# dfm/george

Measured on NVIDIA H100. Metric: gp.compute+log_likelihood N-points/sec, higher is better.
Workload: dtype f64

## Files before the change

george_b200/csrc/hodlr.cu:

```cuda
#include <algorithm>
#include <cmath>
#include <cstdlib>
#include <cstring>
#include <vector>

#include "common.cuh"
#include "hodlr_kernels.cuh"
#include "hodlr_lu.cuh"
#include "hodlr_aca2.cuh"
#include "hodlr_leaf.cuh"
#include "linalg.cuh"
#include "kernel_eval.cuh"

namespace bgp {
int upload_program(const DevProgram& P, DevBuf<DevProgram>& buf, cudaStream_t s);
int kmat_grad_contract_launch(const DevProgram* dprog, int nd, int np, const unsigned* which_dev, const double* x,
                              int64_t n, const double* M, int64_t ldm, const double* alpha, double ca, double cm,
                              double* g_dev, double* diag_dev, DevBuf<double>& scratch, cudaStream_t s);
int fill_identity_launch(double* A, int64_t n, cudaStream_t s);
int64_t grad_slab_partial_size(int64_t n, int64_t c, int np);
int64_t grad_slab_tile_size(int64_t n, int np);
int kmat_grad_slab_launch(const DevProgram* dprog, int nd, int np, const unsigned* which_dev, const double* x, int64_t n,
                          const double* W, int64_t j0, int64_t nc, int64_t jlo, int64_t jhi, const double* alpha,
                          double* partial, double* tile_part, double* diag_dev, cudaStream_t s);
// ... 94 lines not shown
  DevBuf<int> d_idx, d_piv_rows, d_piv_cols, d_ticket, d_chain_done, d_ncols_by_depth;
  DevBuf<uint32_t> d_chain_state;
  DevBuf<A2Node> d_a2nodes;
  DevBuf<A2State> d_a2states;
  DevBuf<MT19937> d_a2rngs;
  DevBuf<A2EPart> d_epart;
  DevBuf<int> d_cand, d_cand_k, d_cand_words, d_cand_L, d_cand_next, d_cand_live, d_cchunk_node, d_rchunk_node, d_nactive;
  DevBuf<double> d_node_box;
  DevBuf<double2> d_cand_xu, d_gbox, d_cbox;
  DevBuf<unsigned long long> d_cmax, d_stats;
  DevBuf<int4> d_work;
  DevBuf<int> d_work_count, d_iter;
  AcaGraphKey aca_key;
  cudaGraph_t aca_graph = nullptr;
  cudaGraphExec_t aca_exec = nullptr;
  cudaStream_t sC = nullptr;
  bool profile = false;
  std::vector<cudaEvent_t> prof_events;
  double prof[12] = {0, 0, 0, 0, 0, 0, 0, 0, 0, 0, 0, 0};
  uint64_t draw_paths[4] = {0, 0, 0, 0};
  uint64_t eval_units[2] = {0, 0};
  DevBuf<double> d_vpart, d_upart, d_vmax;
  int aca_iters = 0;
  size_t w_cap = 0;

  double t_ms[5] = {0, 0, 0, 0, 0};
  double grad_t[4] = {0, 0, 0, 0};
  double work[6] = {0, 0, 0, 0, 0, 0};
};

static int ensure_streams(bgp_hodlr* h) {
  if (!h->sA) {
    BGP_CUDA(cudaStreamCreateWithFlags(&h->sA, cudaStreamNonBlocking));
    BGP_CUDA(cudaStreamCreateWithFlags(&h->sB, cudaStreamNonBlocking));
    for (int i = 0; i < 8; ++i) BGP_CUDA(cudaEventCreate(&h->ev[i]));
  }
  return BGP_OK;
}

static void build_tree(bgp_hodlr* h, int start, int size, int dir, int parent, int depth) {
  HNode nd;
  nd.start = start; nd.size = size; nd.half = size / 2; nd.dir = dir; nd.parent = parent; nd.depth = depth;
  nd.is_leaf = !(nd.half >= h->opts.min_size);
  nd.slot = 0;
  const int id = (int)h->nodes.size();
  h->nodes.push_back(nd);
  if (!nd.is_leaf) {
    build_tree(h, start, nd.half, 0, id, depth + 1);
    build_tree(h, start + nd.half, size - nd.half, 1, id, depth + 1);
  }
}

static int hodlr_solve_dev(bgp_hodlr* h, double* b, int64_t nrhs, int64_t ldb, cudaStream_t s, int part,
                           int64_t eye_row0 = -1);
static int hodlr_exchange_finish(bgp_hodlr* h);

static bool host_exchange(const bgp_hodlr* h) {
  return h->opts.shard_count > 1 &&
         !(comm_ready() && comm_world() == h->opts.shard_count && comm_rank() == h->opts.shard_rank);
}

static int reject_host_exchange(const bgp_hodlr* h, const char* what) {
  if (!host_exchange(h)) return BGP_OK;
  set_error("%s is not available on a host-exchange shard (shard %d of %d without a matching communicator): use "
            "bgp_hodlr_solve_local_dev / bgp_hodlr_solve_top_dev", what, h->opts.shard_rank, h->opts.shard_count);
  return BGP_ERR_INVALID;
}
// ... 198 lines not shown
  BGP_TRY(h->d_cand_L.reserve((size_t)cand_total, s));
  BGP_TRY(h->d_cand_next.reserve((size_t)cand_total, s));
  BGP_TRY(h->d_cand_live.reserve((size_t)cand_total, s));
  BGP_TRY(h->d_node_box.reserve((size_t)2 * nn, s));
  BGP_TRY(h->d_cmax.reserve((size_t)cand_total, s));
  BGP_TRY(h->d_epart.reserve((size_t)std::max(ncc, 1) * A2_NSUB, s));
  BGP_TRY(h->d_cchunk_node.reserve(ncc, s));
  BGP_TRY(h->d_rchunk_node.reserve(nrc, s));
  BGP_TRY(h->d_vpart.reserve((size_t)ncc * A2_NSUB * (capmax + 1), s));
  BGP_TRY(h->d_upart.reserve((size_t)nrc * A2_NSUB * (capmax + 1), s));
  const bool cull = shape_has_bound(h->prog.shape) && !getenv("BGP_NO_CULL");
  if (cull) {
    BGP_TRY(h->d_vmax.reserve((size_t)ncc * A2_NGROUP, s));
    BGP_TRY(h->d_cand_xu.reserve((size_t)cand_total, s));
    BGP_TRY(h->d_gbox.reserve((size_t)ncc * A2_NGROUP, s));
    BGP_TRY(h->d_cbox.reserve((size_t)ncc, s));
  }
  BGP_TRY(h->d_nactive.reserve(2, s));
  int n_top = 0;
  for (int i = 0; i < nn; ++i) n_top += hn[i].is_top;
  BGP_TRY(h->d_stats.reserve(A2_NSTATS, s));
  int64_t work_cap = 0;
  for (int i = 0; i < nn; ++i) {
    const int big = (hn[i].bmax + A2_CG * A2_ITEM_CB - 1) / (A2_CG * A2_ITEM_CB);
    const int small = (std::min(hn[i].bmax, 256) + A2_CG - 1) / A2_CG;
    work_cap += (int64_t)hn[i].n_cchunks * std::max(big, small);
  }
  BGP_TRY(h->d_work.reserve((size_t)(2 * work_cap), s));
  BGP_TRY(h->d_work_count.reserve(4, s));
  BGP_TRY(h->d_iter.reserve(1, s));
  BGP_CUDA(cudaMemsetAsync(h->d_iter.p, 0, sizeof(int), s));
  BGP_CUDA(cudaMemsetAsync(h->d_work_count.p, 0, sizeof(int) * 4, s));
  BGP_CUDA(cudaMemsetAsync(h->d_stats.p, 0, sizeof(unsigned long long) * A2_NSTATS, s));
  BGP_CUDA(cudaMemcpyAsync(h->d_a2nodes.p, hn.data(), sizeof(A2Node) * nn, cudaMemcpyHostToDevice, s));
  BGP_CUDA(cudaMemcpyAsync(h->d_cchunk_node.p, cchunk_node.data(), sizeof(int) * ncc, cudaMemcpyHostToDevice, s));
  BGP_CUDA(cudaMemcpyAsync(h->d_rchunk_node.p, rchunk_node.data(), sizeof(int) * nrc, cudaMemcpyHostToDevice, s));
  BGP_CUDA(cudaMemcpyAsync(h->d_nactive.p, &nn, sizeof(int), cudaMemcpyHostToDevice, s));
  A2Args a;
  memset(&a, 0, sizeof(a));
  a.prog = h->d_prog.p; a.x = h->d_x.p; a.nodes = h->d_a2nodes.p; a.states = h->d_a2states.p; a.rngs = h->d_a2rngs.p; a.n_nodes = nn;
  a.tol = h->opts.tol; a.seed = (uint32_t)h->opts.seed; a.exhaust_mode = h->opts.exhaust_mode;
  a.idx_ws = h->d_idx.p; a.piv_rows = h->d_piv_rows.p; a.piv_cols = h->d_piv_cols.p;
  a.cand = h->d_cand.p; a.cand_k = h->d_cand_k.p; a.cand_words = h->d_cand_words.p; a.cmax = h->d_cmax.p; a.epart = h->d_epart.p;
  a.cchunk_node = h->d_cchunk_node.p; a.rchunk_node = h->d_rchunk_node.p; a.vpart = h->d_vpart.p; a.upart = h->d_upart.p;
  a.vmax = cull ? h->d_vmax.p : nullptr;
  a.cand_xu = cull ? h->d_cand_xu.p : nullptr;
  a.gbox = cull ? h->d_gbox.p : nullptr;
  a.cbox = cull ? h->d_cbox.p : nullptr;
  a.cand_L = h->d_cand_L.p; a.cand_next = h->d_cand_next.p; a.cand_live = h->d_cand_live.p; a.node_box = h->d_node_box.p;
  a.capmax = capmax; a.n_active = h->d_nactive.p; a.stats = h->d_stats.p;
  a.work = h->d_work.p; a.work_count = h->d_work_count.p; a.work_cursor = h->d_work_count.p + 2; a.work_cap = (int)work_cap; a.iter_ptr = h->d_iter.p;
  a.shard_rank = dist_top ? h->opts.shard_rank : 0; a.shard_count = dist_top ? h->opts.shard_count : 1;
  if (dist_top) BGP_CUDA(cudaMemcpyAsync(h->d_nactive.p + 1, &n_top, sizeof(int), cudaMemcpyHostToDevice, s));
  cudaFuncSetAttribute(a2_init_kernel, cudaFuncAttributeMaxDynamicSharedMemorySize, (int)sizeof(A2NodeSmem));
    cudaFuncSetAttribute(a2_decide_kernel, cudaFuncAttributeMaxDynamicSharedMemorySize, (int)sizeof(A2NodeSmem));
    cudaFuncSetAttribute(a2_finish_kernel, cudaFuncAttributeMaxDynamicSharedMemorySize, (int)sizeof(A2NodeSmem));
  a2_init_kernel<<<nn, A2_NODE_THREADS, sizeof(A2NodeSmem), s>>>(a);
  BGP_LAUNCH_CHECK();
  int active = nn, iters = 0;
  int eval_minb = A2_EVAL_MINB_DEFAULT;
  if (const char* e = getenv("BGP_EVAL_MINB")) eval_minb = atoi(e) == 3 ? 3 : 2;
  const int eval_grid = num_sms() * 6;
  auto launch_iteration = [&](cudaStream_t st, cudaGraphConditionalHandle hnd, int use_hnd, int it_prof) -> int {
    auto mark = [&](int slot) -> int {
      if (it_prof < 0) return BGP_OK;
      const size_t need = (size_t)7 * (it_prof + 1);
      while (h->prof_events.size() < need) {
        cudaEvent_t e;
        BGP_CUDA(cudaEventCreate(&e));
        h->prof_events.push_back(e);
      }
      BGP_CUDA(cudaEventRecord(h->prof_events[(size_t)7 * it_prof + slot], st));
      return BGP_OK;
    };
    BGP_TRY(mark(0));
    a2_eval_launch(h->prog.shape, dim3(eval_grid), st, a, eval_minb);
    BGP_LAUNCH_CHECK();
    BGP_TRY(mark(1));
    a2_decide_kernel<<<nn, A2_NODE_THREADS, sizeof(A2NodeSmem), st>>>(a);
    BGP_LAUNCH_CHECK();
    BGP_TRY(mark(2));
    a2_vrow_launch(h->prog.shape, dim3(ncc, A2_NSUB), st, a);
    BGP_LAUNCH_CHECK();
    BGP_TRY(mark(3));
    a2_pivot_kernel<<<nn, 32, 0, st>>>(a);
    BGP_LAUNCH_CHECK();
    BGP_TRY(mark(4));
    a2_vnorm_ucol_launch(h->prog.shape, dim3(ncc + nrc, A2_NSUB), st, a, ncc);
    BGP_LAUNCH_CHECK();
// ... 195 lines not shown
    hleaves[i].start = nd.start; hleaves[i].size = nd.size; hleaves[i].depth = nd.depth; hleaves[i]._pad = 0;
    hleaves[i].off = loff;
    loff += (int64_t)nd.size * nd.size;
    h->max_leaf = std::max(h->max_leaf, nd.size);
  }
  if (h->max_leaf > LS_MAX_LEAF) {
    set_error("leaf size %d too large: the leaf solve handles at most %d rows (N=%lld, min_size=%d); lower min_size",
              h->max_leaf, LS_MAX_LEAF, (long long)n, o.min_size);
    return BGP_ERR_INVALID;
  }
  BGP_TRY(h->d_leaves.reserve(std::max(nl, 1), sA));
  BGP_TRY(h->d_L.reserve((size_t)std::max<int64_t>(loff, 1), sA));
  BGP_TRY(h->d_leaf_logdet.reserve(std::max(nl, 1), sA));
  if (nl) {
    BGP_CUDA(cudaMemcpyAsync(h->d_leaves.p, hleaves.data(), sizeof(LeafDesc) * nl, cudaMemcpyHostToDevice, sA));
    const char* lf_env = getenv("BGP_LEAF_FACTOR");
    const bool generic = lf_env && strcmp(lf_env, "generic") == 0;
    if (h->max_leaf <= LF_MAX_LEAF && !generic) {
      leaf_factor_launch(h->prog.shape, nl, h->max_leaf, sA, h->d_prog.p, h->d_x.p, h->d_diag.p, h->d_leaves.p, h->d_L.p,
                         h->d_leaf_logdet.p);
    } else {
      leaf_build_factor_kernel<<<nl, LEAF_THREADS, 0, sA>>>(h->d_prog.p, h->d_x.p, h->d_diag.p, h->d_leaves.p, h->d_L.p,
                                                            h->d_leaf_logdet.p);
    }
    BGP_LAUNCH_CHECK();
  }
  BGP_CUDA(cudaEventRecord(h->ev[1], sA));

  std::vector<AcaDesc> hdesc;
  std::vector<int> desc_node;
  std::vector<AcaOut> houts;
  int64_t idx_total = 0, piv_total = 0;
  int nint = 0;
  BGP_CUDA(cudaStreamWaitEvent(sB, h->ev[1], 0));
  for (int attempt = 0;; ++attempt) {
    int vcols_set[2] = {0, 0};
    for (auto& L : h->levels) { L.vcol = vcols_set[L.set]; vcols_set[L.set] += L.cap; }
    h->top.vcols = vcols_set[0]; h->loc.vcols = vcols_set[1];
    h->vcols = vcols_set[0] + vcols_set[1];
    hdesc.clear(); desc_node.clear();
    h->piv_off.assign(h->nodes.size(), -1);
    idx_total = 0; piv_total = 0; nint = 0;
    for (int l = 0; l < nlev; ++l) {
      for (int id : h->levels[l].nodes) {
        const HNode& nd = h->nodes[id];
        AcaDesc d;
        d.row0 = nd.start + nd.half; d.n_rows = nd.size - nd.half; d.col0 = nd.start; d.n_cols = nd.half;
        d.vcol = h->levels[l].vcol; d.cap = h->levels[l].cap; d.pre_id = id; d.node = nint;
        d.idx_off = idx_total; d.piv_off = piv_total;
        h->piv_off[id] = (int)piv_total;
        idx_total += d.n_rows; piv_total += d.cap;
        hdesc.push_back(d); desc_node.push_back(id);
        nint++;
      }
    }
    std::vector<int> order(nint);
    for (int i = 0; i < nint; ++i) order[i] = i;
    if (o.rng_mode == BGP_RNG_REFERENCE) std::sort(order.begin(), order.end(), [&](int a, int b) { return hdesc[a].pre_id < hdesc[b].pre_id; });
    else std::stable_sort(order.begin(), order.end(), [&](int a, int b) {
      const int ta = h->nodes[hdesc[a].pre_id].top, tb = h->nodes[hdesc[b].pre_id].top;
      if (ta != tb) return ta > tb;
      return hdesc[a].n_rows > hdesc[b].n_rows;
    });
    std::vector<AcaDesc> hdesc_sorted(nint);
    for (int i = 0; i < nint; ++i) hdesc_sorted[i] = hdesc[order[i]];

    {
// ... 1084 lines not shown
```

george_b200/csrc/hodlr_aca2.cuh:

```cuda
#pragma once

#include "hodlr_kernels.cuh"

namespace bgp {

constexpr int A2_CHUNK = 1024;
constexpr int A2_THREADS = 256;
constexpr int A2_NODE_THREADS = 1024;
constexpr int A2_EPT = A2_CHUNK / A2_THREADS;
constexpr int A2_CG = 4;
constexpr int A2_ITEM_CB = 8;
constexpr int A2_BMAX = 8192;
constexpr int A2_EVAL_MINB_DEFAULT = 3;
constexpr int A2_BGROW = 8;
constexpr int A2_NSUB = 4;
constexpr int A2_GROUP = A2_CHUNK / (A2_THREADS / 32);
constexpr int A2_NGROUP = A2_CHUNK / A2_GROUP;
static_assert(A2_NSUB * A2_THREADS == A2_CHUNK, "sub-chunks tile a chunk");
constexpr int A2_HASH = 16384;
static_assert(A2_BMAX <= 65536, "multimap values are 16-bit draw numbers");
constexpr int A2_XWORDS = 64;
constexpr int A2_PUB_BLOCKS = A2_BMAX / (A2_CG * A2_ITEM_CB);
static_assert(256 / A2_CG <= A2_PUB_BLOCKS, "blocks of A2_CG candidates (batches of up to 256 live ones) fit too");

struct A2Node {
  int row0, n_rows, col0, n_cols;
  int vcol, cap, pre_id, node;
  int cchunk0, n_cchunks, rchunk0, n_rchunks;
  int bmax, is_top;
  int64_t idx_off, piv_off, cand_off;
  double* vbase;
  int64_t ld;
};

struct A2State {
  int rank, draws, n_index, fallback, status, active;
  int phase;
  int B, ncand, piv_i, piv_j;
  int end_words;
  int deferred;
  double pivot, norm;
// ... 90 lines not shown
  double* node_box;
  unsigned long long* cmax;
  A2EPart* epart;
  const int* cchunk_node;
  const int* rchunk_node;
  double* vpart;
  double* upart;
  double* vmax;
  double2* cand_xu;
  double2* gbox;
  double2* cbox;
  int capmax;
  int* n_active;
  int4* work;
  int* work_count;
  int* work_cursor;
  int work_cap;
  int* iter_ptr;
  int shard_rank, shard_count;
  unsigned long long* stats;
};
enum {
  A2_PATH_REDO = 4,
  A2_PATH_TRUNCATED = 5,
  A2_PATH_SEQUENTIAL = 6,
  A2_PATH_PARTIAL = 7,
  A2_UNITS_PULLED = 8,
  A2_UNITS_LIVE = 9,
  A2_NSTATS = 10
};

struct A2NodeSmem {
  MT19937 rng;
  int k[A2_BMAX];
  int ol[A2_BMAX];
  int hkey[A2_HASH];
  unsigned short hval[A2_HASH];
  uint32_t raw[A2_BMAX + A2_XWORDS];
  double red[32];
  int redi[32];
  int flag;
  int n_live;
  int extra;
};
static_assert(sizeof(int) * A2_HASH >= sizeof(double) * (3 * A2_PUB_BLOCKS + 1), "a2_generate's per-block ranges fit in hkey");

__device__ __forceinline__ unsigned a2_hash(int pos) { return ((unsigned)pos * 2654435761u) & (A2_HASH - 1); }
__device__ __forceinline__ int a2_prev_writer(const A2NodeSmem& S, int pos, int c) {
  int best = -1;
  unsigned h = a2_hash(pos);
  while (true) {
    const int key = S.hkey[h];
    if (key == -1) break;
    if (key == pos) { const int v = S.hval[h]; if (v < c && v > best) best = v; }
    h = (h + 1) & (A2_HASH - 1);
  }
  return best;
}
__device__ __forceinline__ int a2_next_writer(const A2NodeSmem& S, int pos, int c) {
  int best = 0x7fffffff;
  unsigned h = a2_hash(pos);
  while (true) {
    const int key = S.hkey[h];
    if (key == -1) break;
    if (key == pos) { const int v = S.hval[h]; if (v > c && v < best) best = v; }
    h = (h + 1) & (A2_HASH - 1);
  }
  return best;
// ... 26 lines not shown
  total = 0;
  for (int w = 0; w < nw; ++w) {
    const int t = s_warp[w];
    before += (w < warp) ? t : 0;
    total += t;
  }
  return before + inc - v;
}

__device__ inline void a2_generate(const A2Args& a, A2State& st, A2NodeSmem& S, const A2Node& nd, int nid, int nb) {
  int* __restrict__ index = a.idx_ws + nd.idx_off;
  int* __restrict__ cand = a.cand + nd.cand_off;
  int* __restrict__ cand_k = a.cand_k + nd.cand_off;
  int* __restrict__ words = a.cand_words + nd.cand_off;
  int* __restrict__ cand_L = a.cand_L + nd.cand_off;
  int* __restrict__ cand_next = a.cand_next + nd.cand_off;
  int* __restrict__ live = a.cand_live + nd.cand_off;
  unsigned long long* __restrict__ cmax = a.cmax + nd.cand_off;
  const int n_index = st.n_index;
  int B = min(min(st.B, nd.bmax), n_index);
  MT19937* rng_commit = a.rngs + 2 * (int64_t)nid;
  MT19937* rng_end = rng_commit + 1;
  if (threadIdx.x == 0) { S.flag = 0x7fffffff; S.n_live = 0; S.extra = 0; }
  mt_fill_coop(S.rng, S.raw, B);
  int start = 0;
  bool truncated = false;
  while (true) {
    const int extra = S.extra;
    for (int c = start + threadIdx.x; c < B; c += blockDim.x) {
      const uint32_t srange = (uint32_t)(n_index - c);
      const uint64_t prod = (uint64_t)S.raw[c + extra] * (uint64_t)srange;
      const uint32_t low = (uint32_t)prod;
      if (low < srange && low < (0u - srange) % srange) atomicMin(&S.flag, c);
      S.k[c] = (int)(prod >> 32);
      words[c] = c + 1 + extra;
      cmax[c] = 0ull;
    }
    __syncthreads();
    const int c0 = S.flag;
    if (c0 == 0x7fffffff) break;
    __syncthreads();
    if (threadIdx.x == 0) {
      atomicAdd(a.stats + A2_PATH_REDO, 1ull);
      const uint32_t srange = (uint32_t)(n_index - c0);
      const uint32_t thr = (0u - srange) % srange;
      int e = extra;
      int kk = -1;
      while (e + 1 < A2_XWORDS && c0 + e + 1 < B + extra) {
        ++e;
        const uint64_t prod = (uint64_t)S.raw[c0 + e] * (uint64_t)srange;
        if ((uint32_t)prod >= thr) { kk = (int)(prod >> 32); break; }
      }
      if (kk >= 0) { S.k[c0] = kk; words[c0] = c0 + 1 + e; S.extra = e; S.flag = 0x7fffffff; }
      else S.flag = -1 - c0;
    }
    __syncthreads();
    if (S.flag < 0) {
      const int c0t = -1 - S.flag;
      __syncthreads();
      if (c0t > 0) {
        if (threadIdx.x == 0) atomicAdd(a.stats + A2_PATH_TRUNCATED, 1ull);
        B = c0t; truncated = true; break;
      }
      mt_copy(&S.rng, rng_commit);
      __syncthreads();
      if (threadIdx.x == 0) {
        atomicAdd(a.stats + A2_PATH_SEQUENTIAL, 1ull);
        int w = 0; S.k[0] = mt_uniform(S.rng, (uint32_t)n_index, &w); words[0] = w; cmax[0] = 0ull; S.extra = -1;
      }
      __syncthreads();
      B = 1;
      break;
    }
    {
      const int grown = S.extra - extra;
      mt_fill_coop(S.rng, S.raw + B + extra, grown);
    }
    start = c0 + 1;
  }
  __syncthreads();
  mt_copy(rng_end, &S.rng);
  if (threadIdx.x == 0) {
    st.ncand = B;
    st.end_words = (!truncated && S.extra >= 0 && B > 0 && words[B - 1] == B + S.extra) ? B + S.extra : -1;
  }
  for (int t = threadIdx.x; t < A2_HASH; t += blockDim.x) S.hkey[t] = -1;
  __syncthreads();
  for (int c = threadIdx.x; c < B; c += blockDim.x) {
    const int pos = S.k[c];
    S.ol[c] = index[n_index - 1 - c];
    unsigned h = a2_hash(pos);
    while (atomicCAS(&S.hkey[h], -1, pos) != -1) h = (h + 1) & (A2_HASH - 1);
    S.hval[h] = (unsigned short)c;
  }
  __syncthreads();
  int* wl = reinterpret_cast<int*>(S.raw);
  for (int c = threadIdx.x; c < B; c += blockDim.x) wl[c] = a2_prev_writer(S, n_index - 1 - c, c);
  __syncthreads();
  auto last_value = [&](int c) {
    int w = wl[c];
    while (w >= 0) { c = w; w = wl[c]; }
    return S.ol[c];
  };
  for (int c = threadIdx.x; c < B; c += blockDim.x) {
    const int pos = S.k[c];
    const int wk = a2_prev_writer(S, pos, c);
    const int row = (wk < 0) ? index[pos] : last_value(wk);
    cand[c] = row;
    cand_k[c] = pos;
    cand_L[c] = last_value(c);
    cand_next[c] = a2_next_writer(S, pos, c);
  }
  const bool cull = a.vmax != nullptr;
  const int rank = st.rank;
  if (!cull) {
    for (int c = threadIdx.x; c < B; c += blockDim.x) live[c] = c;
    if (threadIdx.x == 0) S.n_live = B;
  } else {
    const double clo = a.node_box[2 * nid], chi = a.node_box[2 * nid + 1];
    const double* Ucol = nd.vbase + nd.row0;
    const double* xr = a.x + nd.row0;
    constexpr int G = 4;
    for (int t0 = 0; t0 < B; t0 += G * blockDim.x) {
      const int c0 = t0 + threadIdx.x;
      int row[G];
      double xi[G], b[G];
#pragma unroll
      for (int j = 0; j < G; ++j) { const int c = c0 + j * blockDim.x; row[j] = (c < B) ? cand[c] : 0; }
#pragma unroll
      for (int j = 0; j < G; ++j) xi[j] = xr[row[j]];
#pragma unroll
      for (int j = 0; j < G; ++j) b[j] = 0.0;
      for (int q = 0; q < rank; ++q) {
        double u[G];
#pragma unroll
        for (int j = 0; j < G; ++j) u[j] = __ldcg(Ucol + (int64_t)q * nd.ld + row[j]);
#pragma unroll
        for (int j = 0; j < G; ++j) b[j] += fabs(u[j]);
      }
      unsigned keep = 0u;
#pragma unroll
      for (int j = 0; j < G; ++j) {
        const int c = c0 + j * blockDim.x;
        if (c < B) {
          const double bb = b[j] + program_bound(a.prog, fmax(0.0, fmax(clo - xi[j], xi[j] - chi)), fmax(xi[j] - clo, chi - xi[j]));
          if (!(bb * 1.000001 < 1e-14)) keep |= 1u << j;
        }
      }
      const int base = S.n_live;
      int total;
      int pos = base + a2_block_scan(__popc(keep), S.redi, total);
#pragma unroll
      for (int j = 0; j < G; ++j) {
        if (keep & (1u << j)) {
          const int c = c0 + j * blockDim.x;
          live[pos++] = c;
          a.cand_xu[nd.cand_off + c] = make_double2(xi[j], b[j]);
        }
      }
      if (threadIdx.x == 0) S.n_live = base + total;
      __syncthreads();
    }
  }
  __syncthreads();
  {
    int n_live = S.n_live;
    const bool defer = (B == 1 && n_live == 1);
    if (threadIdx.x == 0) st.deferred = defer ? 1 : 0;
    if (defer) n_live = 0;
    const int ipc = (n_live <= 256) ? A2_CG : A2_CG * A2_ITEM_CB;
    const int per_chunk = (n_live + ipc - 1) / ipc;
    int my_chunks = nd.n_cchunks;
    const bool split = nd.is_top && a.shard_count > 1;
    if (split) my_chunks = (nd.n_cchunks - a.shard_rank + a.shard_count - 1) / a.shard_count;
    const int n_items = my_chunks * per_chunk;
    int4* work_next = a.work + (int64_t)nb * a.work_cap;
    auto item = [&](int t) {
      const int ci = t / per_chunk, pi = t % per_chunk;
      const int lc = split ? (a.shard_rank + ci * a.shard_count) : ci;
      const int c0 = pi * ipc;
      return make_int4(nd.cchunk0 + lc, c0, min(ipc, n_live - c0), nid);
    };
    __syncthreads();
    if (!cull) {
      if (threadIdx.x == 0) {
        S.flag = n_items ? atomicAdd(a.work_count + nb, n_items) : 0;
        if (S.flag + n_items > a.work_cap) st.status = 2;
      }
      __syncthreads();
      const int base = S.flag;
      for (int t = threadIdx.x; t < n_items; t += blockDim.x)
        if (base + t < a.work_cap) work_next[base + t] = item(t);
    } else {
      double* s_blo = reinterpret_cast<double*>((reinterpret_cast<uintptr_t>(S.hkey) + 7) & ~uintptr_t(7));
      double* s_bhi = s_blo + A2_PUB_BLOCKS;
      double* s_bu = s_bhi + A2_PUB_BLOCKS;
      for (int p0 = 0; p0 < per_chunk * ipc; p0 += blockDim.x) {
        const int p = p0 + threadIdx.x;
        double lo = __longlong_as_double(0x7ff0000000000000ll), hi = -lo, u = 0.0;
        bool bnan = false;
        if (p < n_live) {
          const double2 xu = a.cand_xu[nd.cand_off + live[p]];
          lo = hi = xu.x; u = xu.y;
          bnan = (xu.x != xu.x) || (xu.y != xu.y);
        }
        for (int o = 1; o < ipc; o <<= 1) {
          lo = fmin(lo, __shfl_xor_sync(0xffffffffu, lo, o));
          hi = fmax(hi, __shfl_xor_sync(0xffffffffu, hi, o));
          u = fmax(u, __shfl_xor_sync(0xffffffffu, u, o));
          bnan |= __shfl_xor_sync(0xffffffffu, (int)bnan, o) != 0;
        }
        if (bnan) lo = hi = u = __longlong_as_double(0x7ff8000000000000ll);
        if (p % ipc == 0 && p < n_live) { s_blo[p / ipc] = lo; s_bhi[p / ipc] = hi; s_bu[p / ipc] = u; }
      }
      __syncthreads();
      constexpr int R = 32;
      for (int r0 = 0; r0 < n_items; r0 += R * blockDim.x) {
        unsigned keep = 0u;
        for (int k = 0; k < R; ++k) {
          const int t = r0 + k * blockDim.x + threadIdx.x;
          if (t >= n_items) break;
          const int4 w = item(t);
          const int lc = w.x - nd.cchunk0, pi = w.y / ipc;
          const double2 cb = __ldcg(a.cbox + w.x);
          double vm = 0.0;
          bool vnan = false;
          for (int g = 0; g < A2_NGROUP && lc * A2_CHUNK + g * A2_GROUP < nd.n_cols; ++g) {
            const double v = __ldcg(a.vmax + ((int64_t)w.x * A2_NGROUP + g));
            vm = fmax(vm, v); vnan |= (v != v);
          }
          if (vnan) vm = __longlong_as_double(0x7ff8000000000000ll);
          const double lo = s_blo[pi], hi = s_bhi[pi];
          const double bb = program_bound(a.prog, fmax(0.0, fmax(cb.x - hi, lo - cb.y)), fmax(hi - cb.x, cb.y - lo)) + s_bu[pi] * vm;
          if (!(bb * 1.00001 < 1e-14)) keep |= 1u << k;
        }
        int total;
        const int off = a2_block_scan(__popc(keep), S.redi, total);
        if (threadIdx.x == 0) {
          S.flag = total ? atomicAdd(a.work_count + nb, total) : 0;
          if (S.flag + total > a.work_cap) st.status = 2;
        }
        __syncthreads();
        int q = S.flag + off;
        for (int k = 0; k < R; ++k) {
          if (keep & (1u << k)) {
            if (q < a.work_cap) work_next[q] = item(r0 + k * blockDim.x + threadIdx.x);
            ++q;
          }
        }
        __syncthreads();
      }
    }
  }
  __syncthreads();
}

__global__ void __launch_bounds__(A2_NODE_THREADS) a2_init_kernel(A2Args a) {
  extern __shared__ __align__(16) unsigned char a2_smem_raw[];
  A2NodeSmem& S = *reinterpret_cast<A2NodeSmem*>(a2_smem_raw);
  const int nid = blockIdx.x;
  const A2Node nd = a.nodes[nid];
  A2State& st = a.states[nid];
  int* index = a.idx_ws + nd.idx_off;
  for (int n = threadIdx.x; n < nd.n_rows; n += blockDim.x) index[n] = n;
  if (threadIdx.x == 0) {
    mt_seed(S.rng, node_seed(a.seed, nd.pre_id));
    st.rank = 0; st.draws = 0; st.n_index = nd.n_rows; st.fallback = 0; st.status = 0; st.active = 1;
    st.phase = A2_SELECT; st.B = 4; st.norm = 0.0; st.pivot = 0.0; st.piv_i = 0; st.piv_j = 0; st.ncand = 0;
  }
  __syncthreads();
  mt_copy(a.rngs + 2 * (int64_t)nid, &S.rng);
  __syncthreads();
  if (nd.cap <= 0) {
    if (threadIdx.x == 0) { st.status = 1; st.phase = A2_DONE; st.active = 0; { atomicSub(a.n_active, 1); if (nd.is_top) atomicSub(a.n_active + 1, 1); } }
    return;
  }
  if (a.vmax) {
    double lo = __longlong_as_double(0x7ff0000000000000ll), hi = -lo;
    bool has_nan = false;
    for (int n = threadIdx.x; n < nd.n_cols; n += blockDim.x) { const double xv = a.x[nd.col0 + n]; lo = fmin(lo, xv); hi = fmax(hi, xv); has_nan |= (xv != xv); }
    lo = -block_max_signed(-lo, S.red);
    hi = block_max_signed(hi, S.red);
    if (__syncthreads_or(has_nan)) lo = hi = __longlong_as_double(0x7ff8000000000000ll);
    if (threadIdx.x == 0) { a.node_box[2 * nid] = lo; a.node_box[2 * nid + 1] = hi; }
    const int lane = threadIdx.x & 31, nw = blockDim.x >> 5;
    for (int g = threadIdx.x >> 5; g < nd.n_cchunks * A2_NGROUP; g += nw) {
      const int w_lo = g * A2_GROUP;
      const int w_n = min(A2_GROUP, nd.n_cols - w_lo);
      if (w_n <= 0) break;
      double glo = __longlong_as_double(0x7ff0000000000000ll), ghi = -glo;
// ... 154 lines not shown
  constexpr bool CULL = shape_has_bound(SHAPE);
  unsigned long long n_eval = 0ull, n_fma = 0ull;
  unsigned n_pulled = 0u, n_live_units = 0u;
  int* cursor = a.work_cursor + buf;
  if (blockIdx.x == 0 && threadIdx.x == 0) a.work_cursor[buf ^ 1] = 0;
  const int n_units = n_items * A2_NGROUP;
  while (true) {
    int u = 0;
    if ((threadIdx.x & 31) == 0) u = atomicAdd(cursor, 1);
    u = __shfl_sync(0xffffffffu, u, 0);
    if (u >= n_units) break;
    ++n_pulled;
    const int4 w = items[u / A2_NGROUP];
    const int grp = u % A2_NGROUP;
    const A2Node& nd = a.nodes[w.w];
    const int rank = a.states[w.w].rank;
    if constexpr (SHAPE == BGP_SHAPE_GENERIC) a2_eval_body<decltype(fn), false>(a, nd, rank, w.x, w.y, w.z, P.ndim, fn, grp, n_eval, n_fma, n_live_units);
    else a2_eval_body<decltype(fn), CULL>(a, nd, rank, w.x, w.y, w.z, 1, fn, grp, n_eval, n_fma, n_live_units);
  }
  if ((threadIdx.x & 31) == 0 && n_eval) { atomicAdd(a.stats + 3, n_eval); atomicAdd(a.stats + 1, n_fma); }
  if ((threadIdx.x & 31) == 0 && n_pulled) {
    atomicAdd(a.stats + A2_UNITS_PULLED, (unsigned long long)n_pulled);
    atomicAdd(a.stats + A2_UNITS_LIVE, (unsigned long long)n_live_units);
  }
}
inline void a2_eval_launch(int shape, dim3 grid, cudaStream_t s, const A2Args& a, int minb) {
  if (minb == 3 && shape != BGP_SHAPE_GENERIC) {
    BGP_SHAPE_SWITCH(shape, (a2_eval_kernel<SHAPE, (SHAPE == BGP_SHAPE_GENERIC ? 2 : 3)><<<grid, A2_THREADS, 0, s>>>(a)));
  } else {
    BGP_SHAPE_SWITCH(shape, (a2_eval_kernel<SHAPE, 2><<<grid, A2_THREADS, 0, s>>>(a)));
  }
}

__global__ void __launch_bounds__(A2_NODE_THREADS) a2_decide_kernel(A2Args a) {
  extern __shared__ __align__(16) unsigned char a2_smem_raw[];
  A2NodeSmem& S = *reinterpret_cast<A2NodeSmem*>(a2_smem_raw);
  __shared__ int s_winner;
  const int nid = blockIdx.x;
  A2State& st = a.states[nid];
  if (st.phase != A2_SELECT || !st.active) return;
  const A2Node nd = a.nodes[nid];
  const int ncand = st.ncand;
  int* cand = a.cand + nd.cand_off;
  int* cand_k = a.cand_k + nd.cand_off;
  int* words = a.cand_words + nd.cand_off;
  int* index = a.idx_ws + nd.idx_off;
  const int lane = threadIdx.x & 31, warp = threadIdx.x >> 5;
  if (threadIdx.x == 0) {
    s_winner = 0x7fffffff;
  }
  __syncthreads();
  const bool deferred = st.deferred != 0;
  if (deferred) {
    if (threadIdx.x == 0) { s_winner = 0; atomicAdd(a.stats + 3, (unsigned long long)nd.n_cols); }
  } else {
    const unsigned long long* cmax = a.cmax + nd.cand_off;
    int mine = 0x7fffffff;
    for (int c = threadIdx.x; c < ncand; c += blockDim.x) {
      const double m = __longlong_as_double((long long)cmax[c]);
      if (!(m < 1e-14)) { mine = c; break; }
    }
    if (mine != 0x7fffffff) atomicMin(&s_winner, mine);
  }
  __syncthreads();
  const int p = s_winner;
  {
    MT19937* rng_commit = a.rngs + 2 * (int64_t)nid;
// ... 250 lines not shown
  if (r_lo >= nd.n_rows) return;
  if constexpr (SHAPE == BGP_SHAPE_GENERIC) stage_program(&P, a.prog);
  const int ndim = a.prog->ndim;
  const int rank = st.rank;
  const int r_n = min(A2_THREADS, nd.n_rows - r_lo);
  double* Vcols = nd.vbase;
  const int j = st.piv_j;
  for (int q = threadIdx.x; q < ndim; q += A2_THREADS) s_x[q] = a.x[(int64_t)(nd.col0 + j) * ndim + q];
  __syncthreads();
  const auto fn = ShapeEval<SHAPE>::make(&P, a.prog);
  const int n = threadIdx.x;
  const bool act = n < r_n;
  const int nn = act ? n : 0;
  const double val = a2_resid_entry(fn, a.x + (int64_t)(nd.row0 + r_lo + nn) * ndim, s_x, rank, Vcols + nd.row0 + r_lo + nn, nd.ld,
                                    Vcols + nd.col0 + j, s_vr, act);
  double un2 = 0.0;
  if (act) {
    Vcols[(int64_t)rank * nd.ld + nd.row0 + r_lo + n] = val;
    un2 = val * val;
  }
  s_u[n] = act ? val : 0.0;
  un2 = block_sum(un2, red);
  double* part = a.upart + ((int64_t)chunk * A2_NSUB + sub) * (a.capmax + 1);
  if (threadIdx.x == 0) part[0] = un2;
  a2_partial_dots(Vcols + nd.row0 + r_lo, nd.ld, rank, s_u, r_n, part);
}
inline void a2_vrow_launch(int shape, dim3 grid, cudaStream_t s, const A2Args& a) {
  BGP_SHAPE_SWITCH(shape, (a2_vrow_kernel<SHAPE><<<grid, A2_THREADS, 0, s>>>(a)));
}
inline void a2_vnorm_ucol_launch(int shape, dim3 grid, cudaStream_t s, const A2Args& a, int ncc) {
  BGP_SHAPE_SWITCH(shape, (a2_vnorm_ucol_kernel<SHAPE><<<grid, A2_THREADS, 0, s>>>(a, ncc)));
}

__global__ void __launch_bounds__(A2_NODE_THREADS) a2_finish_kernel(A2Args a) {
  extern __shared__ __align__(16) unsigned char a2_smem_raw[];
  A2NodeSmem& S = *reinterpret_cast<A2NodeSmem*>(a2_smem_raw);
  __shared__ int s_done;
  const int nid = blockIdx.x;
  A2State& st = a.states[nid];
  if (!st.active) return;
  if (st.phase == A2_LATE_REJECT) {
    const A2Node nd = a.nodes[nid];
    __syncthreads();
    if (threadIdx.x == 0) {
      st.B = min(A2_BGROW * st.B, A2_BMAX);
      if (st.n_index == 0) {
        st.fallback = 1;
        st.phase = A2_DONE; st.active = 0;
        { atomicSub(a.n_active, 1); if (nd.is_top) atomicSub(a.n_active + 1, 1); }
      } else {
        st.phase = A2_SELECT;
      }
    }
    __syncthreads();
    if (st.phase == A2_DONE) return;
    mt_copy(&S.rng, a.rngs + 2 * (int64_t)nid);
    __syncthreads();
    a2_generate(a, st, S, nd, nid, (*a.iter_ptr + 1) & 1);
    return;
  }
  if (st.phase != A2_ACCEPT) return;
  const A2Node nd = a.nodes[nid];
  const int rank = st.rank;
  double vn2 = 0.0, un2 = 0.0;
  const int nvs = (nd.n_cols + A2_THREADS - 1) / A2_THREADS, nus = (nd.n_rows + A2_THREADS - 1) / A2_THREADS;
  const double* vp0 = a.vpart + (int64_t)nd.cchunk0 * A2_NSUB * (a.capmax + 1);
  const double* up0 = a.upart + (int64_t)nd.rchunk0 * A2_NSUB * (a.capmax + 1);
  for (int c = threadIdx.x; c < nvs; c += blockDim.x) vn2 += vp0[(int64_t)c * (a.capmax + 1)];
  for (int c = threadIdx.x; c < nus; c += blockDim.x) un2 += up0[(int64_t)c * (a.capmax + 1)];
  vn2 = block_sum(vn2, S.red);
  un2 = block_sum(un2, S.red);
  double vdot = 0.0, udot = 0.0;
  for (int k = threadIdx.x; k < rank; k += blockDim.x) {
    double sv = 0.0, su = 0.0;
    for (int c = 0; c < nvs; ++c) sv += vp0[(int64_t)c * (a.capmax + 1) + 1 + k];
    for (int c = 0; c < nus; ++c) su += up0[(int64_t)c * (a.capmax + 1) + 1 + k];
    vdot = fmax(vdot, fabs(sv));
    udot = fmax(udot, fabs(su));
  }
  vdot = block_max(vdot, S.red);
  udot = block_max(udot, S.red);
  mt_copy(&S.rng, a.rngs + 2 * (int64_t)nid);
  if (threadIdx.x == 0) {
    a.piv_rows[nd.piv_off + rank] = st.piv_i;
    a.piv_cols[nd.piv_off + rank] = st.piv_j;
    const int new_rank = rank + 1;
    st.rank = new_rank;
    const int max_rank = min(nd.n_rows, nd.n_cols);
    bool done = false;
    if (new_rank >= max_rank) done = true;
    else {
      const double rowcol = un2 * vn2;
      if (rowcol < a.tol * a.tol * st.norm) done = true;
      else {
        st.norm += rowcol;
        if (new_rank > 1) st.norm += 2.0 * udot + 2.0 * vdot;
        if (new_rank >= nd.cap) { st.status = 1; done = true; }
        else if (st.n_index == 0) { st.fallback = 1; done = true; }
      }
    }
    if (done) {
      st.phase = A2_DONE; st.active = 0;
      { atomicSub(a.n_active, 1); if (nd.is_top) atomicSub(a.n_active + 1, 1); }
    } else {
// ... 50 lines not shown
```

Baseline: 22.70 million.

## Halve ACA node-kernel block size, keep 1024-thread layout, drop smem arrays

The per-node ACA kernels drop from 1024 to 512 threads with a minBlocks=2 launch bound. Their loops and reductions emulate the original 1024-thread item layout in segments, so the order of work items and the floating-point summation stays the same. Two shared-memory arrays (k, ol) are removed in favour of reading from global cand_k and index, which shrinks smem so two CTAs can fit per SM. The change also gives stream sB the highest priority, lets sB wait on an earlier event outside reference RNG mode, and zeroes vmax when culling. In exchange it adds more register pressure per thread and more global reads.

```diff
diff --git a/george_b200/csrc/hodlr.cu b/george_b200/csrc/hodlr.cu
--- a/george_b200/csrc/hodlr.cu
+++ b/george_b200/csrc/hodlr.cu
@@ -150,7 +150,9 @@
 static int ensure_streams(bgp_hodlr* h) {
   if (!h->sA) {
     BGP_CUDA(cudaStreamCreateWithFlags(&h->sA, cudaStreamNonBlocking));
-    BGP_CUDA(cudaStreamCreateWithFlags(&h->sB, cudaStreamNonBlocking));
+    int prio_least = 0, prio_greatest = 0;
+    BGP_CUDA(cudaDeviceGetStreamPriorityRange(&prio_least, &prio_greatest));
+    BGP_CUDA(cudaStreamCreateWithPriority(&h->sB, cudaStreamNonBlocking, prio_greatest));
     for (int i = 0; i < 8; ++i) BGP_CUDA(cudaEventCreate(&h->ev[i]));
   }
   return BGP_OK;
@@ -415,6 +417,7 @@
   BGP_CUDA(cudaMemsetAsync(h->d_iter.p, 0, sizeof(int), s));
   BGP_CUDA(cudaMemsetAsync(h->d_work_count.p, 0, sizeof(int) * 4, s));
   BGP_CUDA(cudaMemsetAsync(h->d_stats.p, 0, sizeof(unsigned long long) * A2_NSTATS, s));
+  if (cull) BGP_CUDA(cudaMemsetAsync(h->d_vmax.p, 0, sizeof(double) * (size_t)ncc * A2_NGROUP, s));
   BGP_CUDA(cudaMemcpyAsync(h->d_a2nodes.p, hn.data(), sizeof(A2Node) * nn, cudaMemcpyHostToDevice, s));
   BGP_CUDA(cudaMemcpyAsync(h->d_cchunk_node.p, cchunk_node.data(), sizeof(int) * ncc, cudaMemcpyHostToDevice, s));
   BGP_CUDA(cudaMemcpyAsync(h->d_rchunk_node.p, rchunk_node.data(), sizeof(int) * nrc, cudaMemcpyHostToDevice, s));
@@ -436,8 +439,8 @@
   a.shard_rank = dist_top ? h->opts.shard_rank : 0; a.shard_count = dist_top ? h->opts.shard_count : 1;
   if (dist_top) BGP_CUDA(cudaMemcpyAsync(h->d_nactive.p + 1, &n_top, sizeof(int), cudaMemcpyHostToDevice, s));
   cudaFuncSetAttribute(a2_init_kernel, cudaFuncAttributeMaxDynamicSharedMemorySize, (int)sizeof(A2NodeSmem));
-    cudaFuncSetAttribute(a2_decide_kernel, cudaFuncAttributeMaxDynamicSharedMemorySize, (int)sizeof(A2NodeSmem));
-    cudaFuncSetAttribute(a2_finish_kernel, cudaFuncAttributeMaxDynamicSharedMemorySize, (int)sizeof(A2NodeSmem));
+  cudaFuncSetAttribute(a2_decide_kernel, cudaFuncAttributeMaxDynamicSharedMemorySize, (int)sizeof(A2NodeSmem));
+  cudaFuncSetAttribute(a2_finish_kernel, cudaFuncAttributeMaxDynamicSharedMemorySize, (int)sizeof(A2NodeSmem));
   a2_init_kernel<<<nn, A2_NODE_THREADS, sizeof(A2NodeSmem), s>>>(a);
   BGP_LAUNCH_CHECK();
   int active = nn, iters = 0;
@@ -699,7 +702,7 @@
   std::vector<AcaOut> houts;
   int64_t idx_total = 0, piv_total = 0;
   int nint = 0;
-  BGP_CUDA(cudaStreamWaitEvent(sB, h->ev[1], 0));
+  BGP_CUDA(cudaStreamWaitEvent(sB, h->ev[o.rng_mode == BGP_RNG_REFERENCE ? 1 : 0], 0));
   for (int attempt = 0;; ++attempt) {
     int vcols_set[2] = {0, 0};
     for (auto& L : h->levels) { L.vcol = vcols_set[L.set]; vcols_set[L.set] += L.cap; }
diff --git a/george_b200/csrc/hodlr_aca2.cuh b/george_b200/csrc/hodlr_aca2.cuh
--- a/george_b200/csrc/hodlr_aca2.cuh
+++ b/george_b200/csrc/hodlr_aca2.cuh
@@ -6,7 +6,9 @@
 
 constexpr int A2_CHUNK = 1024;
 constexpr int A2_THREADS = 256;
-constexpr int A2_NODE_THREADS = 1024;
+constexpr int A2_NODE_THREADS = 512;
+constexpr int A2_LAYOUT_THREADS = 1024;
+static_assert(A2_LAYOUT_THREADS % A2_NODE_THREADS == 0 && A2_LAYOUT_THREADS == 32 * 32, "layout = whole CTAs, 32 warps");
 constexpr int A2_EPT = A2_CHUNK / A2_THREADS;
 constexpr int A2_CG = 4;
 constexpr int A2_ITEM_CB = 8;
@@ -163,8 +165,6 @@
 
 struct A2NodeSmem {
   MT19937 rng;
-  int k[A2_BMAX];
-  int ol[A2_BMAX];
   int hkey[A2_HASH];
   unsigned short hval[A2_HASH];
   uint32_t raw[A2_BMAX + A2_XWORDS];
@@ -257,7 +257,7 @@
       const uint64_t prod = (uint64_t)S.raw[c + extra] * (uint64_t)srange;
       const uint32_t low = (uint32_t)prod;
       if (low < srange && low < (0u - srange) % srange) atomicMin(&S.flag, c);
-      S.k[c] = (int)(prod >> 32);
+      cand_k[c] = (int)(prod >> 32);
       words[c] = c + 1 + extra;
       cmax[c] = 0ull;
     }
@@ -276,7 +276,7 @@
         const uint64_t prod = (uint64_t)S.raw[c0 + e] * (uint64_t)srange;
         if ((uint32_t)prod >= thr) { kk = (int)(prod >> 32); break; }
       }
-      if (kk >= 0) { S.k[c0] = kk; words[c0] = c0 + 1 + e; S.extra = e; S.flag = 0x7fffffff; }
+      if (kk >= 0) { cand_k[c0] = kk; words[c0] = c0 + 1 + e; S.extra = e; S.flag = 0x7fffffff; }
       else S.flag = -1 - c0;
     }
     __syncthreads();
@@ -291,7 +291,7 @@
       __syncthreads();
       if (threadIdx.x == 0) {
         atomicAdd(a.stats + A2_PATH_SEQUENTIAL, 1ull);
-        int w = 0; S.k[0] = mt_uniform(S.rng, (uint32_t)n_index, &w); words[0] = w; cmax[0] = 0ull; S.extra = -1;
+        int w = 0; cand_k[0] = mt_uniform(S.rng, (uint32_t)n_index, &w); words[0] = w; cmax[0] = 0ull; S.extra = -1;
       }
       __syncthreads();
       B = 1;
@@ -312,8 +312,7 @@
   for (int t = threadIdx.x; t < A2_HASH; t += blockDim.x) S.hkey[t] = -1;
   __syncthreads();
   for (int c = threadIdx.x; c < B; c += blockDim.x) {
-    const int pos = S.k[c];
-    S.ol[c] = index[n_index - 1 - c];
+    const int pos = cand_k[c];
     unsigned h = a2_hash(pos);
     while (atomicCAS(&S.hkey[h], -1, pos) != -1) h = (h + 1) & (A2_HASH - 1);
     S.hval[h] = (unsigned short)c;
@@ -325,14 +324,13 @@
   auto last_value = [&](int c) {
     int w = wl[c];
     while (w >= 0) { c = w; w = wl[c]; }
-    return S.ol[c];
+    return index[n_index - 1 - c];
   };
   for (int c = threadIdx.x; c < B; c += blockDim.x) {
-    const int pos = S.k[c];
+    const int pos = cand_k[c];
     const int wk = a2_prev_writer(S, pos, c);
     const int row = (wk < 0) ? index[pos] : last_value(wk);
     cand[c] = row;
-    cand_k[c] = pos;
     cand_L[c] = last_value(c);
     cand_next[c] = a2_next_writer(S, pos, c);
   }
@@ -346,12 +344,14 @@
     const double* Ucol = nd.vbase + nd.row0;
     const double* xr = a.x + nd.row0;
     constexpr int G = 4;
-    for (int t0 = 0; t0 < B; t0 += G * blockDim.x) {
-      const int c0 = t0 + threadIdx.x;
+    constexpr int LT = A2_LAYOUT_THREADS;
+    for (int t0 = 0; t0 < B; t0 += G * LT)
+    for (int v0 = 0; v0 < LT && t0 + v0 < B; v0 += A2_NODE_THREADS) {
+      const int c0 = t0 + v0 + threadIdx.x;
       int row[G];
       double xi[G], b[G];
 #pragma unroll
-      for (int j = 0; j < G; ++j) { const int c = c0 + j * blockDim.x; row[j] = (c < B) ? cand[c] : 0; }
+      for (int j = 0; j < G; ++j) { const int c = c0 + j * LT; row[j] = (c < B) ? cand[c] : 0; }
 #pragma unroll
       for (int j = 0; j < G; ++j) xi[j] = xr[row[j]];
 #pragma unroll
@@ -366,7 +366,7 @@
       unsigned keep = 0u;
 #pragma unroll
       for (int j = 0; j < G; ++j) {
-        const int c = c0 + j * blockDim.x;
+        const int c = c0 + j * LT;
         if (c < B) {
           const double bb = b[j] + program_bound(a.prog, fmax(0.0, fmax(clo - xi[j], xi[j] - chi)), fmax(xi[j] - clo, chi - xi[j]));
           if (!(bb * 1.000001 < 1e-14)) keep |= 1u << j;
@@ -378,7 +378,7 @@
 #pragma unroll
       for (int j = 0; j < G; ++j) {
         if (keep & (1u << j)) {
-          const int c = c0 + j * blockDim.x;
+          const int c = c0 + j * LT;
           live[pos++] = c;
           a.cand_xu[nd.cand_off + c] = make_double2(xi[j], b[j]);
         }
@@ -440,10 +440,14 @@
       }
       __syncthreads();
       constexpr int R = 32;
-      for (int r0 = 0; r0 < n_items; r0 += R * blockDim.x) {
-        unsigned keep = 0u;
+      constexpr int LT = A2_LAYOUT_THREADS, NSEG = A2_LAYOUT_THREADS / A2_NODE_THREADS;
+      for (int r0 = 0; r0 < n_items; r0 += R * LT) {
+        unsigned keep[NSEG];
+#pragma unroll
+        for (int sg = 0; sg < NSEG; ++sg) {
+        keep[sg] = 0u;
         for (int k = 0; k < R; ++k) {
-          const int t = r0 + k * blockDim.x + threadIdx.x;
+          const int t = r0 + k * LT + sg * A2_NODE_THREADS + threadIdx.x;
           if (t >= n_items) break;
           const int4 w = item(t);
           const int lc = w.x - nd.cchunk0, pi = w.y / ipc;
@@ -457,20 +461,29 @@
           if (vnan) vm = __longlong_as_double(0x7ff8000000000000ll);
           const double lo = s_blo[pi], hi = s_bhi[pi];
           const double bb = program_bound(a.prog, fmax(0.0, fmax(cb.x - hi, lo - cb.y)), fmax(hi - cb.x, cb.y - lo)) + s_bu[pi] * vm;
-          if (!(bb * 1.00001 < 1e-14)) keep |= 1u << k;
+          if (!(bb * 1.00001 < 1e-14)) keep[sg] |= 1u << k;
         }
-        int total;
-        const int off = a2_block_scan(__popc(keep), S.redi, total);
+        }
+        int off[NSEG], total = 0;
+#pragma unroll
+        for (int sg = 0; sg < NSEG; ++sg) {
+          int seg_total;
+          off[sg] = total + a2_block_scan(__popc(keep[sg]), S.redi, seg_total);
+          total += seg_total;
+        }
         if (threadIdx.x == 0) {
           S.flag = total ? atomicAdd(a.work_count + nb, total) : 0;
           if (S.flag + total > a.work_cap) st.status = 2;
         }
         __syncthreads();
-        int q = S.flag + off;
-        for (int k = 0; k < R; ++k) {
-          if (keep & (1u << k)) {
-            if (q < a.work_cap) work_next[q] = item(r0 + k * blockDim.x + threadIdx.x);
-            ++q;
+#pragma unroll
+        for (int sg = 0; sg < NSEG; ++sg) {
+          int q = S.flag + off[sg];
+          for (int k = 0; k < R; ++k) {
+            if (keep[sg] & (1u << k)) {
+              if (q < a.work_cap) work_next[q] = item(r0 + k * LT + sg * A2_NODE_THREADS + threadIdx.x);
+              ++q;
+            }
           }
         }
         __syncthreads();
@@ -480,7 +493,7 @@
   __syncthreads();
 }
 
-__global__ void __launch_bounds__(A2_NODE_THREADS) a2_init_kernel(A2Args a) {
+__global__ void __launch_bounds__(A2_NODE_THREADS, 2) a2_init_kernel(A2Args a) {
   extern __shared__ __align__(16) unsigned char a2_smem_raw[];
   A2NodeSmem& S = *reinterpret_cast<A2NodeSmem*>(a2_smem_raw);
   const int nid = blockIdx.x;
@@ -701,7 +714,7 @@
   }
 }
 
-__global__ void __launch_bounds__(A2_NODE_THREADS) a2_decide_kernel(A2Args a) {
+__global__ void __launch_bounds__(A2_NODE_THREADS, 2) a2_decide_kernel(A2Args a) {
   extern __shared__ __align__(16) unsigned char a2_smem_raw[];
   A2NodeSmem& S = *reinterpret_cast<A2NodeSmem*>(a2_smem_raw);
   __shared__ int s_winner;
@@ -1018,7 +1031,25 @@
   BGP_SHAPE_SWITCH(shape, (a2_vnorm_ucol_kernel<SHAPE><<<grid, A2_THREADS, 0, s>>>(a, ncc)));
 }
 
-__global__ void __launch_bounds__(A2_NODE_THREADS) a2_finish_kernel(A2Args a) {
+__device__ __forceinline__ double a2_layout_sum(const double* __restrict__ p, int64_t stride, int n, double* red) {
+  constexpr int NSEG = A2_LAYOUT_THREADS / A2_NODE_THREADS;
+  const int lane = threadIdx.x & 31, w = threadIdx.x >> 5;
+  double part[NSEG];
+#pragma unroll
+  for (int sg = 0; sg < NSEG; ++sg) {
+    double v = 0.0;
+    for (int c = sg * A2_NODE_THREADS + threadIdx.x; c < n; c += A2_LAYOUT_THREADS) v += p[(int64_t)c * stride];
+    part[sg] = warp_sum(v);
+  }
+  __syncthreads();
+  if (lane == 0)
+#pragma unroll
+    for (int sg = 0; sg < NSEG; ++sg) red[sg * (A2_NODE_THREADS / 32) + w] = part[sg];
+  __syncthreads();
+  return warp_sum(red[lane]);
+}
+
+__global__ void __launch_bounds__(A2_NODE_THREADS, 2) a2_finish_kernel(A2Args a) {
   extern __shared__ __align__(16) unsigned char a2_smem_raw[];
   A2NodeSmem& S = *reinterpret_cast<A2NodeSmem*>(a2_smem_raw);
   __shared__ int s_done;
@@ -1048,14 +1079,12 @@
   if (st.phase != A2_ACCEPT) return;
   const A2Node nd = a.nodes[nid];
   const int rank = st.rank;
-  double vn2 = 0.0, un2 = 0.0;
+  double vn2, un2;
   const int nvs = (nd.n_cols + A2_THREADS - 1) / A2_THREADS, nus = (nd.n_rows + A2_THREADS - 1) / A2_THREADS;
   const double* vp0 = a.vpart + (int64_t)nd.cchunk0 * A2_NSUB * (a.capmax + 1);
   const double* up0 = a.upart + (int64_t)nd.rchunk0 * A2_NSUB * (a.capmax + 1);
-  for (int c = threadIdx.x; c < nvs; c += blockDim.x) vn2 += vp0[(int64_t)c * (a.capmax + 1)];
-  for (int c = threadIdx.x; c < nus; c += blockDim.x) un2 += up0[(int64_t)c * (a.capmax + 1)];
-  vn2 = block_sum(vn2, S.red);
-  un2 = block_sum(un2, S.red);
+  vn2 = a2_layout_sum(vp0, a.capmax + 1, nvs, S.red);
+  un2 = a2_layout_sum(up0, a.capmax + 1, nus, S.red);
   double vdot = 0.0, udot = 0.0;
   for (int k = threadIdx.x; k < rank; k += blockDim.x) {
     double sv = 0.0, su = 0.0;
```

After: 23.14 million (median of 6 runs). 1.9% higher.
